# Thitrongdan202/Digital-Watermarking-for-image-Video-using-DCT-SVD-Singular-Value-Decomposition

Hardware: AMD Instinct MI355X
Metric: frames/sec embed+extract @4K Y-channel (higher is better)
Workload: dtype f32

## Files before the change

__graft_entry__.py:

```python
from __future__ import annotations

import importlib
import os
import subprocess
import sys

ROOT = os.path.dirname(os.path.abspath(__file__))
PKG_NAME = "digital-watermarking-for-image-video-using-dct-svd-singular-value-decomposition_amd"
CSRC = os.path.join(ROOT, PKG_NAME, "csrc")
LIB = os.path.join(CSRC, "libwmhip.so")
HARNESS_SRC = os.path.join(ROOT, "tests", "host_harness.cpp")
HARNESS_LIB = os.path.join(ROOT, "tests", "_build", "libwm_hostharness.so")

if ROOT not in sys.path:
    sys.path.insert(0, ROOT)


def _newer(target: str, *sources: str) -> bool:
    if not os.path.exists(target):
        return False
    t = os.path.getmtime(target)
    return all(os.path.getmtime(s) <= t for s in sources if os.path.exists(s))


def _run(cmd):
    r = subprocess.run(cmd, stdout=subprocess.PIPE, stderr=subprocess.STDOUT, text=True)
    if r.returncode != 0:
        raise RuntimeError("build failed: " + " ".join(cmd) + "\n" + r.stdout[-4000:])
    return r.stdout


def build_hip(force: bool = False) -> str:
    units = [os.path.join(CSRC, u) for u in ("wmhip.hip", "wm_ref.hip", "wm_pixel.hip", "wm_route.hip", "wm_enhance.hip")]
    deps = units + [os.path.join(CSRC, "wm_tile_math.h"), os.path.join(CSRC, "wm_enhance_math.h"), os.path.join(CSRC, "wm_internal.h"),
                    os.path.join(CSRC, "wm_jacobi_gfx950.inc"), os.path.join(CSRC, "wm_jacobi_v_gfx950.inc"),
                    os.path.join(CSRC, "wm_completion_tables.inc"), os.path.join(CSRC, "wm_ref_hier.inc"),
                    os.path.join(ROOT, "include", "wmhip.h")]
    if force or not _newer(LIB, *deps):
        hipcc = os.environ.get("HIPCC", "/opt/rocm/bin/hipcc")
        _run([hipcc, "-O3", "--offload-arch=gfx950", "-shared", "-fPIC", "-o", LIB] + units)
    return LIB


NOASM_LIB = os.path.join(ROOT, "tests", "_build", "libwmhip_noasm.so")


def build_hip_noasm(force: bool = False) -> str:
    os.makedirs(os.path.dirname(NOASM_LIB), exist_ok=True)
    units = [os.path.join(CSRC, u) for u in ("wmhip.hip", "wm_ref.hip", "wm_pixel.hip", "wm_route.hip", "wm_enhance.hip")]
    deps = units + [os.path.join(CSRC, "wm_tile_math.h"), os.path.join(CSRC, "wm_enhance_math.h"), os.path.join(CSRC, "wm_internal.h"),
                    os.path.join(CSRC, "wm_completion_tables.inc"), os.path.join(CSRC, "wm_ref_hier.inc"),
                    os.path.join(ROOT, "include", "wmhip.h")]
    if force or not _newer(NOASM_LIB, *deps):
        hipcc = os.environ.get("HIPCC", "/opt/rocm/bin/hipcc")
        _run([hipcc, "-O3", "--offload-arch=gfx950", "-shared", "-fPIC", "-DWM_NO_ASM_JACOBI", "-o", NOASM_LIB] + units)
    return NOASM_LIB


def build_host_harness(force: bool = False) -> str:
    os.makedirs(os.path.dirname(HARNESS_LIB), exist_ok=True)
    srcs = [HARNESS_SRC, os.path.join(CSRC, "wm_tile_math.h"), os.path.join(CSRC, "wm_completion_tables.inc")]
    if force or not _newer(HARNESS_LIB, *srcs):
        _run(["g++", "-O2", "-shared", "-fPIC", "-o", HARNESS_LIB, HARNESS_SRC])
    return HARNESS_LIB


MASK_HARNESS_SRC = os.path.join(ROOT, "tests", "mask_harness.cpp")


def build_mask_harness(sanitize: bool = False, force: bool = False) -> str:
    exe = os.path.join(ROOT, "tests", "_build", "mask_harness_san" if sanitize else "mask_harness")
    os.makedirs(os.path.dirname(exe), exist_ok=True)
    if force or not _newer(exe, MASK_HARNESS_SRC, os.path.join(CSRC, "wm_tile_math.h")):
        flags = ["-O1", "-g", "-fsanitize=address,undefined", "-fno-sanitize-recover=all"] if sanitize else ["-O2"]
        _run(["g++"] + flags + ["-o", exe, MASK_HARNESS_SRC])
    return exe


PAYLOAD_HARNESS_SRC = os.path.join(ROOT, "tests", "payload_harness.cpp")


def build_payload_harness(sanitize: bool = False, force: bool = False) -> str:
    exe = os.path.join(ROOT, "tests", "_build", "payload_harness_san" if sanitize else "payload_harness")
    os.makedirs(os.path.dirname(exe), exist_ok=True)
    if force or not _newer(exe, PAYLOAD_HARNESS_SRC, os.path.join(CSRC, "wm_tile_math.h")):
        flags = ["-O1", "-g", "-fsanitize=address,undefined", "-fno-sanitize-recover=all"] if sanitize else ["-O2"]
        _run(["g++"] + flags + ["-o", exe, PAYLOAD_HARNESS_SRC])
    return exe


PAYLOAD_DITHER_HARNESS_SRC = os.path.join(ROOT, "tests", "payload_dither_harness.cpp")


def build_payload_dither_harness(sanitize: bool = False, force: bool = False) -> str:
    exe = os.path.join(ROOT, "tests", "_build", "payload_dither_harness_san" if sanitize else "payload_dither_harness")
    os.makedirs(os.path.dirname(exe), exist_ok=True)
    if force or not _newer(exe, PAYLOAD_DITHER_HARNESS_SRC, os.path.join(CSRC, "wm_tile_math.h")):
        flags = ["-O1", "-g", "-fsanitize=address,undefined", "-fno-sanitize-recover=all"] if sanitize else ["-O2"]
        _run(["g++"] + flags + ["-o", exe, PAYLOAD_DITHER_HARNESS_SRC])
    return exe


PAYLOAD_SYNC_HARNESS_SRC = os.path.join(ROOT, "tests", "payload_sync_harness.cpp")


def build_payload_sync_harness(sanitize: bool = False, force: bool = False) -> str:
    exe = os.path.join(ROOT, "tests", "_build", "payload_sync_harness_san" if sanitize else "payload_sync_harness")
    os.makedirs(os.path.dirname(exe), exist_ok=True)
    if force or not _newer(exe, PAYLOAD_SYNC_HARNESS_SRC, os.path.join(CSRC, "wm_tile_math.h")):
        flags = ["-O1", "-g", "-fsanitize=address,undefined", "-fno-sanitize-recover=all"] if sanitize else ["-O2"]
        _run(["g++"] + flags + ["-o", exe, PAYLOAD_SYNC_HARNESS_SRC])
    return exe


def build() -> None:
    build_hip()
    build_hip_noasm()
    build_host_harness()
    build_mask_harness()
    build_mask_harness(sanitize=True)
# ... 49 lines not shown
```

digital-watermarking-for-image-video-using-dct-svd-singular-value-decomposition_amd/csrc/wm_jacobi_gfx950.inc:

```
__device__ __forceinline__ unsigned long long jacobi_cols_gfx950(const uint32_t (&lo)[8], const uint32_t (&hi)[8],
                                                                 wm::v2f (&a)[4][8], float (&n2)[8], const float conv2,
                                                                 const float skip2, const int min_sweeps,
                                                                 const int skip_from) {
  unsigned long long more;
  asm volatile(
      "s_mov_b32 s82, 0\n\t"
      "s_mov_b32 s83, 0x219392ef\n\t"
      "s_mov_b32 s84, %[conv]\n\t"
      "s_mov_b32 s85, %[skip]\n\t"
      "s_mov_b32 s86, %[minsw]\n\t"
      "s_mov_b32 s87, %[skipfrom]\n\t"
      "v_cvt_f32_ubyte0_e32 v40, %[lo0]\n\t"
      "v_cvt_f32_ubyte1_e32 v42, %[lo0]\n\t"
      "v_cvt_f32_ubyte2_e32 v44, %[lo0]\n\t"
      "v_cvt_f32_ubyte3_e32 v46, %[lo0]\n\t"
      "v_cvt_f32_ubyte0_e32 v48, %[hi0]\n\t"
      "v_cvt_f32_ubyte1_e32 v50, %[hi0]\n\t"
      "v_cvt_f32_ubyte2_e32 v52, %[hi0]\n\t"
      "v_cvt_f32_ubyte3_e32 v54, %[hi0]\n\t"
      "v_cvt_f32_ubyte0_e32 v41, %[lo1]\n\t"
      "v_cvt_f32_ubyte1_e32 v43, %[lo1]\n\t"
      "v_cvt_f32_ubyte2_e32 v45, %[lo1]\n\t"
      "v_cvt_f32_ubyte3_e32 v47, %[lo1]\n\t"
      "v_cvt_f32_ubyte0_e32 v49, %[hi1]\n\t"
      "v_cvt_f32_ubyte1_e32 v51, %[hi1]\n\t"
      "v_cvt_f32_ubyte2_e32 v53, %[hi1]\n\t"
      "v_cvt_f32_ubyte3_e32 v55, %[hi1]\n\t"
      "v_cvt_f32_ubyte0_e32 v56, %[lo2]\n\t"
      "v_cvt_f32_ubyte1_e32 v58, %[lo2]\n\t"
      "v_cvt_f32_ubyte2_e32 v60, %[lo2]\n\t"
      "v_cvt_f32_ubyte3_e32 v62, %[lo2]\n\t"
      "v_cvt_f32_ubyte0_e32 v64, %[hi2]\n\t"
      "v_cvt_f32_ubyte1_e32 v66, %[hi2]\n\t"
      "v_cvt_f32_ubyte2_e32 v68, %[hi2]\n\t"
      "v_cvt_f32_ubyte3_e32 v70, %[hi2]\n\t"
      "v_cvt_f32_ubyte0_e32 v57, %[lo3]\n\t"
      "v_cvt_f32_ubyte1_e32 v59, %[lo3]\n\t"
      "v_cvt_f32_ubyte2_e32 v61, %[lo3]\n\t"
      "v_cvt_f32_ubyte3_e32 v63, %[lo3]\n\t"
      "v_cvt_f32_ubyte0_e32 v65, %[hi3]\n\t"
      "v_cvt_f32_ubyte1_e32 v67, %[hi3]\n\t"
      "v_cvt_f32_ubyte2_e32 v69, %[hi3]\n\t"
      "v_cvt_f32_ubyte3_e32 v71, %[hi3]\n\t"
      "v_cvt_f32_ubyte0_e32 v72, %[lo4]\n\t"
      "v_cvt_f32_ubyte1_e32 v74, %[lo4]\n\t"
      "v_cvt_f32_ubyte2_e32 v76, %[lo4]\n\t"
      "v_cvt_f32_ubyte3_e32 v78, %[lo4]\n\t"
      "v_cvt_f32_ubyte0_e32 v80, %[hi4]\n\t"
      "v_cvt_f32_ubyte1_e32 v82, %[hi4]\n\t"
      "v_cvt_f32_ubyte2_e32 v84, %[hi4]\n\t"
      "v_cvt_f32_ubyte3_e32 v86, %[hi4]\n\t"
      "v_cvt_f32_ubyte0_e32 v73, %[lo5]\n\t"
      "v_cvt_f32_ubyte1_e32 v75, %[lo5]\n\t"
      "v_cvt_f32_ubyte2_e32 v77, %[lo5]\n\t"
      "v_cvt_f32_ubyte3_e32 v79, %[lo5]\n\t"
      "v_cvt_f32_ubyte0_e32 v81, %[hi5]\n\t"
      "v_cvt_f32_ubyte1_e32 v83, %[hi5]\n\t"
      "v_cvt_f32_ubyte2_e32 v85, %[hi5]\n\t"
      "v_cvt_f32_ubyte3_e32 v87, %[hi5]\n\t"
      "v_cvt_f32_ubyte0_e32 v88, %[lo6]\n\t"
      "v_cvt_f32_ubyte1_e32 v90, %[lo6]\n\t"
      "v_cvt_f32_ubyte2_e32 v92, %[lo6]\n\t"
      "v_cvt_f32_ubyte3_e32 v94, %[lo6]\n\t"
      "v_cvt_f32_ubyte0_e32 v96, %[hi6]\n\t"
      "v_cvt_f32_ubyte1_e32 v98, %[hi6]\n\t"
      "v_cvt_f32_ubyte2_e32 v100, %[hi6]\n\t"
      "v_cvt_f32_ubyte3_e32 v102, %[hi6]\n\t"
      "v_cvt_f32_ubyte0_e32 v89, %[lo7]\n\t"
      "v_cvt_f32_ubyte1_e32 v91, %[lo7]\n\t"
      "v_cvt_f32_ubyte2_e32 v93, %[lo7]\n\t"
      "v_cvt_f32_ubyte3_e32 v95, %[lo7]\n\t"
      "v_cvt_f32_ubyte0_e32 v97, %[hi7]\n\t"
      "v_cvt_f32_ubyte1_e32 v99, %[hi7]\n\t"
      "v_cvt_f32_ubyte2_e32 v101, %[hi7]\n\t"
      "v_cvt_f32_ubyte3_e32 v103, %[hi7]\n\t"
      "v_pk_mul_f32 v[120:121], v[40:41], v[40:41]\n\t"
      "v_pk_mul_f32 v[122:123], v[56:57], v[56:57]\n\t"
      "v_pk_mul_f32 v[124:125], v[72:73], v[72:73]\n\t"
      "v_pk_mul_f32 v[126:127], v[88:89], v[88:89]\n\t"
      "v_pk_fma_f32 v[120:121], v[42:43], v[42:43], v[120:121]\n\t"
      "v_pk_fma_f32 v[122:123], v[58:59], v[58:59], v[122:123]\n\t"
      "v_pk_fma_f32 v[124:125], v[74:75], v[74:75], v[124:125]\n\t"
      "v_pk_fma_f32 v[126:127], v[90:91], v[90:91], v[126:127]\n\t"
      "v_pk_fma_f32 v[120:121], v[44:45], v[44:45], v[120:121]\n\t"
      "v_pk_fma_f32 v[122:123], v[60:61], v[60:61], v[122:123]\n\t"
      "v_pk_fma_f32 v[124:125], v[76:77], v[76:77], v[124:125]\n\t"
      "v_pk_fma_f32 v[126:127], v[92:93], v[92:93], v[126:127]\n\t"
      "v_pk_fma_f32 v[120:121], v[46:47], v[46:47], v[120:121]\n\t"
      "v_pk_fma_f32 v[122:123], v[62:63], v[62:63], v[122:123]\n\t"
      "v_pk_fma_f32 v[124:125], v[78:79], v[78:79], v[124:125]\n\t"
      "v_pk_fma_f32 v[126:127], v[94:95], v[94:95], v[126:127]\n\t"
      "v_pk_fma_f32 v[120:121], v[48:49], v[48:49], v[120:121]\n\t"
      "v_pk_fma_f32 v[122:123], v[64:65], v[64:65], v[122:123]\n\t"
      "v_pk_fma_f32 v[124:125], v[80:81], v[80:81], v[124:125]\n\t"
      "v_pk_fma_f32 v[126:127], v[96:97], v[96:97], v[126:127]\n\t"
      "v_pk_fma_f32 v[120:121], v[50:51], v[50:51], v[120:121]\n\t"
      "v_pk_fma_f32 v[122:123], v[66:67], v[66:67], v[122:123]\n\t"
      "v_pk_fma_f32 v[124:125], v[82:83], v[82:83], v[124:125]\n\t"
      "v_pk_fma_f32 v[126:127], v[98:99], v[98:99], v[126:127]\n\t"
      "v_pk_fma_f32 v[120:121], v[52:53], v[52:53], v[120:121]\n\t"
      "v_pk_fma_f32 v[122:123], v[68:69], v[68:69], v[122:123]\n\t"
      "v_pk_fma_f32 v[124:125], v[84:85], v[84:85], v[124:125]\n\t"
      "v_pk_fma_f32 v[126:127], v[100:101], v[100:101], v[126:127]\n\t"
      "v_pk_fma_f32 v[120:121], v[54:55], v[54:55], v[120:121]\n\t"
      "v_pk_fma_f32 v[122:123], v[70:71], v[70:71], v[122:123]\n\t"
      "v_pk_fma_f32 v[124:125], v[86:87], v[86:87], v[124:125]\n\t"
      "v_pk_fma_f32 v[126:127], v[102:103], v[102:103], v[126:127]\n\t"
      "v_max3_f32 v112, v120, v121, v122\n\t"
      "v_max3_f32 v113, v123, v124, v125\n\t"
      "v_max3_f32 v112, v126, v127, v112\n\t"
      "s_mov_b64 s[94:95], 0\n\t"
      "v_max_f32_e32 v112, v112, v113\n\t"
      "v_mov_b32_e32 v113, 0xf149f2ca\n\t"
      "v_cmp_eq_f32_e64 s[92:93], v120, v112\n\t"
      "s_andn2_b64 s[96:97], s[92:93], s[94:95]\n\t"
      "s_or_b64 s[94:95], s[94:95], s[92:93]\n\t"
      "v_cndmask_b32_e64 v120, v120, v113, s[96:97]\n\t"
      "v_cmp_eq_f32_e64 s[92:93], v121, v112\n\t"
      "s_andn2_b64 s[96:97], s[92:93], s[94:95]\n\t"
      "s_or_b64 s[94:95], s[94:95], s[92:93]\n\t"
      "v_cndmask_b32_e64 v121, v121, v113, s[96:97]\n\t"
      "v_cndmask_b32_e64 v104, v40, v41, s[96:97]\n\t"
      "v_cndmask_b32_e64 v105, v42, v43, s[96:97]\n\t"
      "v_cndmask_b32_e64 v106, v44, v45, s[96:97]\n\t"
      "v_cndmask_b32_e64 v107, v46, v47, s[96:97]\n\t"
      "v_cndmask_b32_e64 v108, v48, v49, s[96:97]\n\t"
      "v_cndmask_b32_e64 v109, v50, v51, s[96:97]\n\t"
      "v_cndmask_b32_e64 v110, v52, v53, s[96:97]\n\t"
      "v_cndmask_b32_e64 v111, v54, v55, s[96:97]\n\t"
      "v_cmp_eq_f32_e64 s[92:93], v122, v112\n\t"
      "s_andn2_b64 s[96:97], s[92:93], s[94:95]\n\t"
      "s_or_b64 s[94:95], s[94:95], s[92:93]\n\t"
      "v_cndmask_b32_e64 v122, v122, v113, s[96:97]\n\t"
      "v_cndmask_b32_e64 v104, v104, v56, s[96:97]\n\t"
      "v_cndmask_b32_e64 v105, v105, v58, s[96:97]\n\t"
      "v_cndmask_b32_e64 v106, v106, v60, s[96:97]\n\t"
      "v_cndmask_b32_e64 v107, v107, v62, s[96:97]\n\t"
      "v_cndmask_b32_e64 v108, v108, v64, s[96:97]\n\t"
      "v_cndmask_b32_e64 v109, v109, v66, s[96:97]\n\t"
      "v_cndmask_b32_e64 v110, v110, v68, s[96:97]\n\t"
      "v_cndmask_b32_e64 v111, v111, v70, s[96:97]\n\t"
      "v_cmp_eq_f32_e64 s[92:93], v123, v112\n\t"
      "s_andn2_b64 s[96:97], s[92:93], s[94:95]\n\t"
      "s_or_b64 s[94:95], s[94:95], s[92:93]\n\t"
      "v_cndmask_b32_e64 v123, v123, v113, s[96:97]\n\t"
      "v_cndmask_b32_e64 v104, v104, v57, s[96:97]\n\t"
      "v_cndmask_b32_e64 v105, v105, v59, s[96:97]\n\t"
      "v_cndmask_b32_e64 v106, v106, v61, s[96:97]\n\t"
      "v_cndmask_b32_e64 v107, v107, v63, s[96:97]\n\t"
      "v_cndmask_b32_e64 v108, v108, v65, s[96:97]\n\t"
      "v_cndmask_b32_e64 v109, v109, v67, s[96:97]\n\t"
      "v_cndmask_b32_e64 v110, v110, v69, s[96:97]\n\t"
      "v_cndmask_b32_e64 v111, v111, v71, s[96:97]\n\t"
      "v_cmp_eq_f32_e64 s[92:93], v124, v112\n\t"
      "s_andn2_b64 s[96:97], s[92:93], s[94:95]\n\t"
      "s_or_b64 s[94:95], s[94:95], s[92:93]\n\t"
      "v_cndmask_b32_e64 v124, v124, v113, s[96:97]\n\t"
      "v_cndmask_b32_e64 v104, v104, v72, s[96:97]\n\t"
      "v_cndmask_b32_e64 v105, v105, v74, s[96:97]\n\t"
      "v_cndmask_b32_e64 v106, v106, v76, s[96:97]\n\t"
      "v_cndmask_b32_e64 v107, v107, v78, s[96:97]\n\t"
      "v_cndmask_b32_e64 v108, v108, v80, s[96:97]\n\t"
      "v_cndmask_b32_e64 v109, v109, v82, s[96:97]\n\t"
      "v_cndmask_b32_e64 v110, v110, v84, s[96:97]\n\t"
      "v_cndmask_b32_e64 v111, v111, v86, s[96:97]\n\t"
      "v_cmp_eq_f32_e64 s[92:93], v125, v112\n\t"
      "s_andn2_b64 s[96:97], s[92:93], s[94:95]\n\t"
      "s_or_b64 s[94:95], s[94:95], s[92:93]\n\t"
      "v_cndmask_b32_e64 v125, v125, v113, s[96:97]\n\t"
      "v_cndmask_b32_e64 v104, v104, v73, s[96:97]\n\t"
      "v_cndmask_b32_e64 v105, v105, v75, s[96:97]\n\t"
      "v_cndmask_b32_e64 v106, v106, v77, s[96:97]\n\t"
      "v_cndmask_b32_e64 v107, v107, v79, s[96:97]\n\t"
      "v_cndmask_b32_e64 v108, v108, v81, s[96:97]\n\t"
      "v_cndmask_b32_e64 v109, v109, v83, s[96:97]\n\t"
      "v_cndmask_b32_e64 v110, v110, v85, s[96:97]\n\t"
      "v_cndmask_b32_e64 v111, v111, v87, s[96:97]\n\t"
      "v_cmp_eq_f32_e64 s[92:93], v126, v112\n\t"
      "s_andn2_b64 s[96:97], s[92:93], s[94:95]\n\t"
      "s_or_b64 s[94:95], s[94:95], s[92:93]\n\t"
      "v_cndmask_b32_e64 v126, v126, v113, s[96:97]\n\t"
      "v_cndmask_b32_e64 v104, v104, v88, s[96:97]\n\t"
      "v_cndmask_b32_e64 v105, v105, v90, s[96:97]\n\t"
      "v_cndmask_b32_e64 v106, v106, v92, s[96:97]\n\t"
      "v_cndmask_b32_e64 v107, v107, v94, s[96:97]\n\t"
      "v_cndmask_b32_e64 v108, v108, v96, s[96:97]\n\t"
      "v_cndmask_b32_e64 v109, v109, v98, s[96:97]\n\t"
      "v_cndmask_b32_e64 v110, v110, v100, s[96:97]\n\t"
      "v_cndmask_b32_e64 v111, v111, v102, s[96:97]\n\t"
      "v_cmp_eq_f32_e64 s[92:93], v127, v112\n\t"
// ... 4791 lines not shown
```

digital-watermarking-for-image-video-using-dct-svd-singular-value-decomposition_amd/csrc/wm_tile_math.h:

```cpp
#pragma once
#include <stdint.h>
#include <math.h>

#if defined(__HIPCC__)
#define WM_HD __host__ __device__ __forceinline__
#else
#define WM_HD inline
#endif

namespace wm {

WM_HD float frcp(float x) {
#if defined(__HIP_DEVICE_COMPILE__)
  return __builtin_amdgcn_rcpf(x);
#else
  return 1.0f / x;
#endif
}
WM_HD float frsq(float x) {
#if defined(__HIP_DEVICE_COMPILE__)
  return __builtin_amdgcn_rsqf(x);
#else
  return 1.0f / sqrtf(x);
#endif
}
WM_HD float fsqrt(float x) {
#if defined(__HIP_DEVICE_COMPILE__)
  return __builtin_amdgcn_sqrtf(x);
#else
  return sqrtf(x);
#endif
}
WM_HD float ffma(float a, float b, float c) {
#if defined(__HIP_DEVICE_COMPILE__)
  return __builtin_fmaf(a, b, c);
#else
  return fmaf(a, b, c);
#endif
}
WM_HD bool wave_any(bool p) {
#if defined(__HIP_DEVICE_COMPILE__)
  return __builtin_amdgcn_ballot_w64(p) != 0ull;
#else
  return p;
#endif
}

constexpr float C1 = 0.49039264020161522f;
constexpr float C2 = 0.46193976625564337f;
constexpr float C3 = 0.41573480615127262f;
constexpr float C4 = 0.35355339059327379f;
constexpr float C5 = 0.27778511650980114f;
constexpr float C6 = 0.19134171618254492f;
constexpr float C7 = 0.09754516100806417f;

WM_HD void dct8(float& x0, float& x1, float& x2, float& x3,
                float& x4, float& x5, float& x6, float& x7) {
  const float s0 = x0 + x7, s1 = x1 + x6, s2 = x2 + x5, s3 = x3 + x4;
  const float d0 = x0 - x7, d1 = x1 - x6, d2 = x2 - x5, d3 = x3 - x4;
  const float e0 = s0 + s3, e1 = s1 + s2, e2 = s0 - s3, e3 = s1 - s2;
  x0 = C4 * (e0 + e1);
  x4 = C4 * (e0 - e1);
  x2 = ffma(C2, e2, C6 * e3);
  x6 = ffma(C6, e2, -C2 * e3);
  x1 = ffma(C1, d0, ffma(C3, d1, ffma(C5, d2, C7 * d3)));
  x3 = ffma(C3, d0, ffma(-C7, d1, ffma(-C1, d2, -C5 * d3)));
  x5 = ffma(C5, d0, ffma(-C1, d1, ffma(C7, d2, C3 * d3)));
  x7 = ffma(C7, d0, ffma(-C5, d1, ffma(C3, d2, -C1 * d3)));
}

WM_HD void idct8(float& x0, float& x1, float& x2, float& x3,
                 float& x4, float& x5, float& x6, float& x7) {
  const float p = C4 * (x0 + x4), q = C4 * (x0 - x4);
  const float r = ffma(C2, x2, C6 * x6), t = ffma(C6, x2, -C2 * x6);
  const float e0 = p + r, e3 = p - r, e1 = q + t, e2 = q - t;
  const float o0 = ffma(C1, x1, ffma(C3, x3, ffma(C5, x5, C7 * x7)));
  const float o1 = ffma(C3, x1, ffma(-C7, x3, ffma(-C1, x5, -C5 * x7)));
  const float o2 = ffma(C5, x1, ffma(-C1, x3, ffma(C7, x5, C3 * x7)));
  const float o3 = ffma(C7, x1, ffma(-C5, x3, ffma(C3, x5, -C1 * x7)));
  x0 = e0 + o0; x7 = e0 - o0;
  x1 = e1 + o1; x6 = e1 - o1;
  x2 = e2 + o2; x5 = e2 - o2;
  x3 = e3 + o3; x4 = e3 - o3;
}

WM_HD void dct8x8(float (&a)[8][8]) {
#pragma unroll
  for (int c = 0; c < 8; ++c)
    dct8(a[0][c], a[1][c], a[2][c], a[3][c], a[4][c], a[5][c], a[6][c], a[7][c]);
#pragma unroll
  for (int r = 0; r < 8; ++r)
    dct8(a[r][0], a[r][1], a[r][2], a[r][3], a[r][4], a[r][5], a[r][6], a[r][7]);
}
WM_HD void idct8x8(float (&a)[8][8]) {
#pragma unroll
  for (int r = 0; r < 8; ++r)
    idct8(a[r][0], a[r][1], a[r][2], a[r][3], a[r][4], a[r][5], a[r][6], a[r][7]);
#pragma unroll
  for (int c = 0; c < 8; ++c)
    idct8(a[0][c], a[1][c], a[2][c], a[3][c], a[4][c], a[5][c], a[6][c], a[7][c]);
}

constexpr float JAC_TOL2 = 1e-15f;
constexpr float JAC_CONV2 = 1e-7f;
constexpr int JAC_MAX_SWEEPS = 12;
constexpr int JAC_DEFI_FROM = 6;
constexpr float JAC_CONV2_SIGMA = 1e-2f;
constexpr float JAC_MOVE2 = 1e-6f;
constexpr float JAC_SKIP2 = 1e-12f;

template <bool WITH_V>
WM_HD void jacobi_rot(float (&a)[8][8], float (&v)[8][8], float (&n2)[8],
                      const int p, const int q, bool& notconv) {
  float g = a[0][p] * a[0][q];
#pragma unroll
  for (int r = 1; r < 8; ++r) g = ffma(a[r][p], a[r][q], g);
  const float al = n2[p], be = n2[q];
  const float ab = al * be, gg = g * g;
  const bool big = gg > JAC_TOL2 * ab;
  notconv = notconv || (gg > JAC_CONV2 * ab);
  const float tau = be - al, g2 = g + g;
  const float h = fsqrt(ffma(tau, tau, g2 * g2));
  float t = g2 * frcp(fabsf(tau) + h);
  t = (tau < 0.0f) ? -t : t;
  t = big ? t : 0.0f;
  const float c = frsq(ffma(t, t, 1.0f)), s = c * t;
  const float tg = t * g;
  const float aln = al - tg, ben = be + tg;
  const bool sw = tau > 0.0f;
  const float C = sw ? s : c, S = sw ? -c : s;
  n2[p] = sw ? ben : aln;
  n2[q] = sw ? aln : ben;
#pragma unroll
  for (int r = 0; r < 8; ++r) {
    const float x = a[r][p], y = a[r][q];
    a[r][p] = ffma(C, x, -S * y);
    a[r][q] = ffma(S, x, C * y);
  }
  if (WITH_V) {
#pragma unroll
    for (int r = 0; r < 8; ++r) {
      const float x = v[r][p], y = v[r][q];
      v[r][p] = ffma(C, x, -S * y);
      v[r][q] = ffma(S, x, C * y);
    }
  }
}

WM_HD void col_norms2(const float (&a)[8][8], float (&n2)[8]) {
#pragma unroll
  for (int c = 0; c < 8; ++c) {
    float s = a[0][c] * a[0][c];
#pragma unroll
    for (int r = 1; r < 8; ++r) s = ffma(a[r][c], a[r][c], s);
    n2[c] = s;
  }
}

template <bool WITH_V>
WM_HD int jacobi_svd8(float (&a)[8][8], float (&v)[8][8], float (&n2)[8], float (&vn2)[8]) {
  if (WITH_V) {
#pragma unroll
    for (int r = 0; r < 8; ++r)
#pragma unroll
      for (int c = 0; c < 8; ++c) v[r][c] = (r == c) ? 1.0f : 0.0f;
  }
  int sweep = 0;
  bool more = true;
  while (more && sweep < JAC_MAX_SWEEPS) {
    col_norms2(a, n2);
    bool notconv = false;
#pragma unroll
    for (int p = 0; p < 7; ++p)
#pragma unroll
      for (int q = p + 1; q < 8; ++q) jacobi_rot<WITH_V>(a, v, n2, p, q, notconv);
    ++sweep;
    more = wave_any(notconv);
  }
  col_norms2(a, n2);
  if (WITH_V) col_norms2(v, vn2);
  else {
#pragma unroll
    for (int c = 0; c < 8; ++c) vn2[c] = 1.0f;
  }
  return more ? -sweep : sweep;
}

typedef float v2f __attribute__((vector_size(8)));

// ... 34 lines not shown
  x3 = e3 + o3; x4 = e3 - o3;
}
WM_HD void dct8x8_to_pk(const float (&a)[8][8], v2f (&b)[4][8]) {
#pragma unroll
  for (int c = 0; c < 8; ++c) {
    float x0 = a[0][c], x1 = a[1][c], x2 = a[2][c], x3 = a[3][c], x4 = a[4][c], x5 = a[5][c], x6 = a[6][c], x7 = a[7][c];
    dct8(x0, x1, x2, x3, x4, x5, x6, x7);
    const v2f p0 = {x0, x1}, p1 = {x2, x3}, p2 = {x4, x5}, p3 = {x6, x7};
    b[0][c] = p0; b[1][c] = p1; b[2][c] = p2; b[3][c] = p3;
  }
#pragma unroll
  for (int rp = 0; rp < 4; ++rp)
    dct8_pk(b[rp][0], b[rp][1], b[rp][2], b[rp][3], b[rp][4], b[rp][5], b[rp][6], b[rp][7]);
}
WM_HD void idct8x8_from_pk(v2f (&b)[4][8], float (&a)[8][8]) {
#pragma unroll
  for (int rp = 0; rp < 4; ++rp)
    idct8_pk(b[rp][0], b[rp][1], b[rp][2], b[rp][3], b[rp][4], b[rp][5], b[rp][6], b[rp][7]);
#pragma unroll
  for (int c = 0; c < 8; ++c) {
    float x0 = b[0][c][0], x1 = b[0][c][1], x2 = b[1][c][0], x3 = b[1][c][1];
    float x4 = b[2][c][0], x5 = b[2][c][1], x6 = b[3][c][0], x7 = b[3][c][1];
    idct8(x0, x1, x2, x3, x4, x5, x6, x7);
    a[0][c] = x0; a[1][c] = x1; a[2][c] = x2; a[3][c] = x3; a[4][c] = x4; a[5][c] = x5; a[6][c] = x6; a[7][c] = x7;
  }
}

template <int HALF>
WM_HD v2f fma2_bcast(const v2f ab, const v2f x, v2f acc) {
#if defined(__HIP_DEVICE_COMPILE__)
  if (HALF == 0) asm("v_pk_fma_f32 %0, %1, %2, %0 op_sel_hi:[0,1,1]" : "+v"(acc) : "v"(ab), "v"(x));
  else asm("v_pk_fma_f32 %0, %1, %2, %0 op_sel:[1,0,0]" : "+v"(acc) : "v"(ab), "v"(x));
  return acc;
#else
  return fma2(splat2(ab[HALF]), x, acc);
#endif
}
template <int HALF>
WM_HD v2f mul2_bcast(const v2f ab, const v2f x) {
#if defined(__HIP_DEVICE_COMPILE__)
  v2f r;
  if (HALF == 0) asm("v_pk_mul_f32 %0, %1, %2 op_sel_hi:[0,1]" : "=v"(r) : "v"(ab), "v"(x));
  else asm("v_pk_mul_f32 %0, %1, %2 op_sel:[1,0]" : "=v"(r) : "v"(ab), "v"(x));
  return r;
#else
  return splat2(ab[HALF]) * x;
#endif
}

constexpr float SIGMA_RATIO_MIN2 = 1e-10f;

template <int CHECK, bool SKIP = false>
WM_HD void jacobi_rot_pk(v2f (&a)[4][8], float (&n2)[8], const int p, const int q, bool& notconv) {
  v2f gv = a[0][p] * a[0][q];
#pragma unroll
  for (int rp = 1; rp < 4; ++rp) gv = fma2(a[rp][p], a[rp][q], gv);
  const float g = gv[0] + gv[1];
  const float al = n2[p], be = n2[q];
  if (CHECK) notconv = notconv || (g * g > (CHECK == 2 ? JAC_CONV2_SIGMA : JAC_CONV2) * (al * be));
  if (SKIP && !wave_any(g * g > JAC_SKIP2 * (al * be))) return;
  const float tau = be - al;
  const float ta = fabsf(tau) + 1e-18f;
  const float g2 = g + g;
  const float ih = frsq(ffma(g2, g2, ta * ta));
  const float x = ffma(0.5f * ta, ih, 0.5f);
  const float rx = frsq(x);
  const float c0 = x * rx;
  const float s0 = (g * ih) * rx;
  const bool sw = tau > 0.0f;
  const float C = sw ? s0 : c0, Sn = sw ? c0 : s0;
  const float w = fabsf((s0 * rx) * g);
  if (CHECK) notconv = notconv || (w * w > (JAC_MOVE2 * fmaxf(al, be)) * n2[0]);
  n2[p] = fmaxf(al, be) + w;
  n2[q] = fminf(al, be) - w;
  const v2f Cv = splat2(C), Sv = splat2(Sn);
#pragma unroll
  for (int rp = 0; rp < 4; ++rp) {
    const v2f X = a[rp][p], Y = a[rp][q];
    a[rp][p] = fma2(Cv, X, Sv * Y);
    a[rp][q] = fma2(Cv, Y, -(Sv * X));
  }
}

WM_HD void jacobi_rot_scaled_pk(v2f (&a)[4][8], float (&n2)[8], float (&w2)[8], const int p, const int q, const bool wave_swaps) {
  v2f gv = a[0][p] * a[0][q];
#pragma unroll
  for (int rp = 1; rp < 4; ++rp) gv = fma2(a[rp][p], a[rp][q], gv);
  const float gt = gv[0] + gv[1];
  const float al = n2[p], be = n2[q];
  const float gg = (gt * (w2[p] * w2[q])) * gt;
  const float tau = be - al;
  const float ta = fabsf(tau) + 1e-18f;
  const float ih = frsq(ffma(gg, 4.0f, ta * ta));
  const float x = ffma(0.5f * ta, ih, 0.5f);
  const float rx = frsq(x);
  const float u = gt * ih;
  const float gh = gg * ih;
  if (!wave_swaps) {
    const float rx2 = rx * rx;
    const float tq = u * w2[p];
    const float v = u * rx2;
    const float w = gh * rx2;
    w2[p] *= x;
    const float tp = v * w2[q];
    w2[q] *= rx2;
    const v2f Tp = splat2(tp), Tq = splat2(-tq);
#pragma unroll
    for (int rp = 0; rp < 4; ++rp) {
      a[rp][p] = fma2(Tp, a[rp][q], a[rp][p]);
      a[rp][q] = fma2(Tq, a[rp][p], a[rp][q]);
    }
    n2[p] = al + w;
    n2[q] = be - w;
  } else {
    const float pq = w2[p] * w2[q];
    const float c0 = x * rx;
    const float r = frsq(pq);
    const float w = (gh * rx) * rx;
    const float s0 = (u * rx) * (pq * r);
    const float rq = w2[q] * r, rp_ = w2[p] * r;
    const bool sw = tau > 0.0f;
    const float Sn = sw ? c0 : s0, C = sw ? s0 : c0;
    const v2f Cv = splat2(C), Sp = splat2(Sn * rq), Sq = splat2(Sn * rp_);
#pragma unroll
    for (int rp = 0; rp < 4; ++rp) {
      const v2f X = a[rp][p], Y = a[rp][q];
      a[rp][p] = fma2(Cv, X, Sp * Y);
      a[rp][q] = fma2(Cv, Y, -(Sq * X));
    }
    n2[p] = fmaxf(al, be) + w;
    n2[q] = fminf(al, be) - w;
  }
}

WM_HD void col_norms2_pk(const v2f (&a)[4][8], float (&n2)[8]) {
#pragma unroll
  for (int c = 0; c < 8; ++c) {
    v2f s = a[0][c] * a[0][c];
#pragma unroll
    for (int rp = 1; rp < 4; ++rp) s = fma2(a[rp][c], a[rp][c], s);
    n2[c] = s[0] + s[1];
  }
}

template <int CHECK, bool SKIP = false>
WM_HD void jacobi_sweep_pk(v2f (&a)[4][8], float (&n2)[8], bool& notconv) {
#pragma unroll
  for (int p = 0; p < 7; ++p)
#pragma unroll
    for (int q = p + 1; q < 8; ++q) jacobi_rot_pk<CHECK, SKIP>(a, n2, p, q, notconv);
}
WM_HD void jacobi_sweep_scaled_pk(v2f (&a)[4][8], float (&n2)[8], float (&w2)[8]) {
#pragma unroll
  for (int p = 0; p < 7; ++p)
#pragma unroll
    for (int q = p + 1; q < 8; ++q) jacobi_rot_scaled_pk(a, n2, w2, p, q, wave_any(n2[q] - n2[p] > 0.0f));
}
WM_HD void col_norms2_scaled_pk(const v2f (&a)[4][8], const float (&w2)[8], float (&n2)[8]) {
  col_norms2_pk(a, n2);
#pragma unroll
  for (int c = 0; c < 8; ++c) n2[c] *= w2[c];
}
WM_HD void fold_scales_pk(v2f (&a)[4][8], const float (&w2)[8]) {
#pragma unroll
  for (int c = 0; c < 8; ++c) {
    const v2f d = splat2(w2[c] * frsq(w2[c]));
#pragma unroll
    for (int rp = 0; rp < 4; ++rp) a[rp][c] = d * a[rp][c];
  }
}

WM_HD float fmax3(const float a, const float b, const float c) { return fmaxf(fmaxf(a, b), c); }
WM_HD void lq_prelude_pk(v2f (&a)[4][8]) {
  v2f rn[4];
#pragma unroll
  for (int c = 0; c < 8; ++c)
#pragma unroll
    for (int rp = 0; rp < 4; ++rp) rn[rp] = (c == 0) ? a[rp][c] * a[rp][c] : fma2(a[rp][c], a[rp][c], rn[rp]);
#pragma unroll
  for (int k = 0; k < 7; ++k) {
    float m = fmax3(rn[0][0], rn[0][1], rn[1][0]);
    const float m2 = fmax3(rn[1][1], rn[2][0], rn[2][1]);
    m = fmaxf(fmax3(rn[3][0], rn[3][1], m), m2);
    float x[8];
    bool found = false;
#pragma unroll
    for (int r = 0; r < 8; ++r) {
      const bool hit = rn[r >> 1][r & 1] == m;
      const bool mine = hit && !found;
      found = found || hit;
      rn[r >> 1][r & 1] = mine ? -1e30f : rn[r >> 1][r & 1];
      if (r) {
#pragma unroll
        for (int c = k; c < 8; ++c) x[c] = mine ? a[r >> 1][c][r & 1] : (r == 1 ? a[0][c][0] : x[c]);
      }
    }
    float t2 = x[7] * x[7];
#pragma unroll
    for (int c = 6; c > k; --c) t2 = ffma(x[c], x[c], t2);
    const float nx2 = ffma(x[k], x[k], t2);
    const float nrm = copysignf(nx2 * frsq(fmaxf(1e-36f, nx2)), x[k]);
    const float vk = x[k] + nrm;
    const float sb = frsq(fmaxf(1e-36f, 0.5f * ffma(vk, vk, t2)));
    x[k] = vk;
#pragma unroll
    for (int c = k; c < 8; ++c) x[c] *= sb;
    v2f w[4];
#pragma unroll
    for (int c = k; c < 8; ++c)
#pragma unroll
      for (int rp = 0; rp < 4; ++rp) w[rp] = (c == k) ? splat2(x[c]) * a[rp][c] : fma2(splat2(x[c]), a[rp][c], w[rp]);
#pragma unroll
    for (int c = k; c < 8; ++c)
#pragma unroll
      for (int rp = 0; rp < 4; ++rp) a[rp][c] = fma2(splat2(x[c]), -w[rp], a[rp][c]);
    if (k < 6) {
#pragma unroll
      for (int rp = 0; rp < 4; ++rp) rn[rp] = fma2(-a[rp][k], a[rp][k], rn[rp]);
    }
  }
}

template <bool SIGMA_ONLY = false>
WM_HD int jacobi_cols_pk(v2f (&a)[4][8], float (&n2)[8]) {
  lq_prelude_pk(a);
  bool notconv = false;
  float w2[8] = {1.0f, 1.0f, 1.0f, 1.0f, 1.0f, 1.0f, 1.0f, 1.0f};
  col_norms2_pk(a, n2);
  jacobi_sweep_scaled_pk(a, n2, w2);
  jacobi_sweep_scaled_pk(a, n2, w2);
  int sweep = 2;
  if (!SIGMA_ONLY) {
    col_norms2_scaled_pk(a, w2, n2);
    jacobi_sweep_scaled_pk(a, n2, w2);
    sweep = 3;
  }
  fold_scales_pk(a, w2);
  bool more = true;
  while (more && sweep < JAC_MAX_SWEEPS) {
    if ((sweep & 1) == 0) col_norms2_pk(a, n2);
    notconv = false;
    if (!SIGMA_ONLY) jacobi_sweep_pk<1, true>(a, n2, notconv);
    else jacobi_sweep_pk<2>(a, n2, notconv);
    ++sweep;
    if (sweep >= JAC_DEFI_FROM && !(n2[7] > SIGMA_RATIO_MIN2 * n2[0])) notconv = false;
    more = wave_any(notconv);
  }
  col_norms2_pk(a, n2);
  return more ? -sweep : sweep;
}

struct RawTile { uint32_t lo[8], hi[8]; };

WM_HD float raw_px(const RawTile& t, const int r, const int c) {
  const uint32_t w = (c < 4) ? t.lo[r] : t.hi[r];
  return (float)((w >> (8 * (c & 3))) & 0xffu);
}
WM_HD void raw_to_pk(const RawTile& t, v2f (&a)[4][8]) {
#pragma unroll
  for (int rp = 0; rp < 4; ++rp)
#pragma unroll
    for (int c = 0; c < 8; ++c) {
      v2f v = {raw_px(t, 2 * rp, c), raw_px(t, 2 * rp + 1, c)};
      a[rp][c] = v;
    }
}
WM_HD void raw_to_f32(const RawTile& t, float (&a)[8][8]) {
#pragma unroll
  for (int r = 0; r < 8; ++r)
#pragma unroll
    for (int c = 0; c < 8; ++c) a[r][c] = raw_px(t, r, c);
}

WM_HD int sigma_tile_pk(const RawTile& t, float (&s)[8]) {
  v2f a[4][8];
  float n2[8];
  raw_to_pk(t, a);
  const int sweeps = jacobi_cols_pk<true>(a, n2);
#pragma unroll
  for (int i = 0; i < 8; ++i) s[i] = fsqrt(n2[i]);
  return sweeps;
}

WM_HD uint32_t quant_u8(float x) {
  x = fminf(fmaxf(x, 0.0f), 255.0f);
  return (uint32_t)x;
}

WM_HD int embed_jacobi_pk(const RawTile& t, v2f (&a)[4][8], float (&n2)[8]) {
  raw_to_pk(t, a);
  return jacobi_cols_pk(a, n2);
}

WM_HD void embed_coeffs_pk(const float (&n2)[8], const float (&sw)[8], const float (&alpha_k)[8],
                           float (&e)[8], float (&sc)[8], bool& deficient) {
  deficient = !(n2[7] > SIGMA_RATIO_MIN2 * n2[0]);
#pragma unroll
  for (int i = 0; i < 8; ++i) {
    const float rs = frsq(fmaxf(n2[i], 1e-30f));
    sc[i] = n2[i] * rs;
    e[i] = (alpha_k[i] * sw[i]) * (rs * rs * rs);
  }
}

template <bool YW>
WM_HD void embed_half_pk(const uint32_t (&w)[8], const v2f (&a)[4][8], const float (&e)[8],
                         uint32_t (&outw)[8], float* yw, const size_t yw_stride) {
#pragma unroll
  for (int r = 0; r < 8; ++r) outw[r] = 0u;
#pragma unroll
  for (int cp = 0; cp < 2; ++cp) {
    const int sh = 16 * cp;
    v2f g[8];
#pragma unroll
    for (int r = 0; r < 8; ++r) {
      const uint32_t ww = w[r] >> sh;
      const v2f x = {(float)(ww & 0xffu), (float)((ww >> 8) & 0xffu)};
#pragma unroll
      for (int i = 0; i < 8; ++i) {
        const v2f ab = a[r >> 1][i];
        if (r == 0) g[i] = mul2_bcast<0>(ab, x);
        else g[i] = (r & 1) ? fma2_bcast<1>(ab, x, g[i]) : fma2_bcast<0>(ab, x, g[i]);
      }
    }
#pragma unroll
    for (int i = 0; i < 8; ++i) g[i] = g[i] * splat2(e[i]);
#pragma unroll
    for (int r = 0; r < 8; ++r) {
      const uint32_t ww = w[r] >> sh;
      v2f y = {(float)(ww & 0xffu), (float)((ww >> 8) & 0xffu)};
#pragma unroll
// ... 683 lines not shown
```

digital-watermarking-for-image-video-using-dct-svd-singular-value-decomposition_amd/csrc/wmhip.hip:

```cpp
#include <hip/hip_runtime.h>
#include <stdio.h>
#include <stdlib.h>
#include <string.h>
#include <new>

#include "wm_internal.h"
#include "wm_tile_math.h"

using namespace wmi;

namespace wmi {

thread_local char g_err[512] = "";

int set_err(int code, const char* fmt, const char* a, const char* b) {
  snprintf(g_err, sizeof(g_err), fmt, a, b);
  return code;
}

int grow(wm_ctx* ctx, void** buf, size_t* have, size_t bytes, const char* what) {
  if (bytes <= *have) return WM_OK;
  if (*buf) {
    WM_HIP(hipStreamSynchronize(ctx->stream));
    WM_HIP(hipFree(*buf));
    *buf = nullptr; *have = 0;
  }
  const size_t mb = (size_t)1 << 20;
  const size_t want = (bytes + mb - 1) / mb * mb;
  if (hipMalloc(buf, want) != hipSuccess) {
    (void)hipGetLastError();
    *buf = nullptr;
    return set_err(WM_ERR_NOMEM, "hipMalloc failed for %s", what);
  }
  *have = want;
  return WM_OK;
}

}

namespace {

constexpr int N_SUMS = 5;

#if !defined(WM_NO_ASM_JACOBI)
#include "wm_jacobi_gfx950.inc"
#endif

__device__ __forceinline__ int sigma_tile_dev(const wm::RawTile& raw, float (&s)[8]) {
#if !defined(WM_NO_ASM_JACOBI)
  wm::v2f a[4][8];
  float n2[8];
  constexpr float SIGMA_SKIP2 = 1e-8f;
  constexpr int SIGMA_SKIP_FROM = 2;
  const unsigned long long more = jacobi_cols_gfx950(raw.lo, raw.hi, a, n2, wm::JAC_CONV2_SIGMA, SIGMA_SKIP2, 3, SIGMA_SKIP_FROM);
#pragma unroll
  for (int i = 0; i < 8; ++i) s[i] = wm::fsqrt(n2[i]);
  return more ? -1 : 1;
#else
  return wm::sigma_tile_pk(raw, s);
#endif
}

template <bool ALIGNED>
__device__ __forceinline__ uint32_t load_px4(const uint8_t* __restrict__ q) {
  if (ALIGNED) return *reinterpret_cast<const uint32_t*>(q);
  return q[0] | (q[1] << 8) | (q[2] << 16) | ((uint32_t)q[3] << 24);
}
template <bool ALIGNED>
__device__ __forceinline__ void store_px4(uint8_t* __restrict__ q, const uint32_t w) {
  if (ALIGNED) { *reinterpret_cast<uint32_t*>(q) = w; return; }
#pragma unroll
  for (int i = 0; i < 4; ++i) q[i] = (uint8_t)(w >> (8 * i));
}
template <bool ALIGNED>
__device__ __forceinline__ void load_px8(const uint8_t* __restrict__ q, uint32_t& lo, uint32_t& hi) {
  if (ALIGNED) { const uint2 w = *reinterpret_cast<const uint2*>(q); lo = w.x; hi = w.y; }
  else { lo = load_px4<false>(q); hi = load_px4<false>(q + 4); }
}
template <bool ALIGNED>
__device__ __forceinline__ void store_px8(uint8_t* __restrict__ q, const uint32_t lo, const uint32_t hi) {
  if (ALIGNED) *reinterpret_cast<uint2*>(q) = make_uint2(lo, hi);
  else { store_px4<false>(q, lo); store_px4<false>(q + 4, hi); }
}

template <bool ALIGNED>
__device__ __forceinline__ void load_raw(const uint8_t* __restrict__ p, const size_t stride, wm::RawTile& t) {
#pragma unroll
  for (int r = 0; r < 8; ++r) load_px8<ALIGNED>(p + r * stride, t.lo[r], t.hi[r]);
}

template <bool ALIGNED>
__device__ __forceinline__ void load_tile_u8(const uint8_t* __restrict__ p, const size_t stride, float (&a)[8][8]) {
#pragma unroll
  for (int r = 0; r < 8; ++r) {
    uint32_t lo, hi;
    load_px8<ALIGNED>(p + r * stride, lo, hi);
    a[r][0] = (float)(lo & 0xffu); a[r][1] = (float)((lo >> 8) & 0xffu);
    a[r][2] = (float)((lo >> 16) & 0xffu); a[r][3] = (float)(lo >> 24);
    a[r][4] = (float)(hi & 0xffu); a[r][5] = (float)((hi >> 8) & 0xffu);
    a[r][6] = (float)((hi >> 16) & 0xffu); a[r][7] = (float)(hi >> 24);
  }
}

template <bool ALIGNED>
__device__ __forceinline__ void store_tile_u8(uint8_t* __restrict__ p, const size_t stride, const float (&a)[8][8]) {
#pragma unroll
  for (int r = 0; r < 8; ++r) {
    const uint32_t lo = wm::quant_u8(a[r][0]) | (wm::quant_u8(a[r][1]) << 8) |
                        (wm::quant_u8(a[r][2]) << 16) | (wm::quant_u8(a[r][3]) << 24);
    const uint32_t hi = wm::quant_u8(a[r][4]) | (wm::quant_u8(a[r][5]) << 8) |
                        (wm::quant_u8(a[r][6]) << 16) | (wm::quant_u8(a[r][7]) << 24);
    store_px8<ALIGNED>(p + r * stride, lo, hi);
  }
}

template <bool ALIGNED>
__device__ __forceinline__ void load_words(const uint8_t* __restrict__ p, const size_t stride, uint32_t (&w)[8]) {
#pragma unroll
  for (int r = 0; r < 8; ++r) w[r] = load_px4<ALIGNED>(p + r * stride);
}
template <bool ALIGNED>
__device__ __forceinline__ void store_words(uint8_t* __restrict__ p, const size_t stride, const uint32_t (&w)[8]) {
#pragma unroll
  for (int r = 0; r < 8; ++r) store_px4<ALIGNED>(p + r * stride, w[r]);
}

template <bool VEC>
__device__ __forceinline__ void load_row8_f32(const float* __restrict__ p, float (&row)[8]) {
  if (VEC) {
    const float4 x = *reinterpret_cast<const float4*>(p);
    const float4 y = *reinterpret_cast<const float4*>(p + 4);
    row[0] = x.x; row[1] = x.y; row[2] = x.z; row[3] = x.w;
    row[4] = y.x; row[5] = y.y; row[6] = y.z; row[7] = y.w;
  } else {
#pragma unroll
    for (int i = 0; i < 8; ++i) row[i] = p[i];
  }
// ... 1844 lines not shown
```

Before: 23420.

## Add sigma-only Jacobi asm kernel and compute initial column norms with integer dot4

Moves the sigma-only tile path to a new generated assembly kernel that returns only the column norms, without producing the rotated matrix. The initial squared column norms are computed directly from packed uint8 pixels with v_dot4_u32_u8 and then converted to float, replacing a chain of packed float FMAs. The portable sigma path now keeps the column scales unfolded through the later sweeps, folds them at a fixed sweep, and uses a reciprocal and an inline convergence test. This aims to cut ALU work and register pressure in the sigma SVD. The risks are a generated include that may not exist at build time and small numeric differences from the changed convergence behaviour.

```diff
diff --git a/__graft_entry__.py b/__graft_entry__.py
--- a/__graft_entry__.py
+++ b/__graft_entry__.py
@@ -33,9 +33,15 @@
 def build_hip(force: bool = False) -> str:
     units = [os.path.join(CSRC, u) for u in ("wmhip.hip", "wm_ref.hip", "wm_pixel.hip", "wm_route.hip", "wm_enhance.hip")]
     deps = units + [os.path.join(CSRC, "wm_tile_math.h"), os.path.join(CSRC, "wm_enhance_math.h"), os.path.join(CSRC, "wm_internal.h"),
-                    os.path.join(CSRC, "wm_jacobi_gfx950.inc"), os.path.join(CSRC, "wm_jacobi_v_gfx950.inc"),
+                    os.path.join(CSRC, "wm_jacobi_gfx950.inc"), os.path.join(CSRC, "wm_jacobi_sigma_gfx950.inc"),
+                    os.path.join(CSRC, "wm_jacobi_v_gfx950.inc"),
                     os.path.join(CSRC, "wm_completion_tables.inc"), os.path.join(CSRC, "wm_ref_hier.inc"),
                     os.path.join(ROOT, "include", "wmhip.h")]
+    sys.path.insert(0, os.path.join(ROOT, "tools"))
+    try:
+        importlib.import_module("gen_jacobi_asm").write_sigma()
+    finally:
+        sys.path.remove(os.path.join(ROOT, "tools"))
     if force or not _newer(LIB, *deps):
         hipcc = os.environ.get("HIPCC", "/opt/rocm/bin/hipcc")
         _run([hipcc, "-O3", "--offload-arch=gfx950", "-shared", "-fPIC", "-o", LIB] + units)
diff --git a/digital-watermarking-for-image-video-using-dct-svd-singular-value-decomposition_amd/csrc/wm_jacobi_gfx950.inc b/digital-watermarking-for-image-video-using-dct-svd-singular-value-decomposition_amd/csrc/wm_jacobi_gfx950.inc
--- a/digital-watermarking-for-image-video-using-dct-svd-singular-value-decomposition_amd/csrc/wm_jacobi_gfx950.inc
+++ b/digital-watermarking-for-image-video-using-dct-svd-singular-value-decomposition_amd/csrc/wm_jacobi_gfx950.inc
@@ -74,38 +74,30 @@
       "v_cvt_f32_ubyte1_e32 v99, %[hi7]\n\t"
       "v_cvt_f32_ubyte2_e32 v101, %[hi7]\n\t"
       "v_cvt_f32_ubyte3_e32 v103, %[hi7]\n\t"
-      "v_pk_mul_f32 v[120:121], v[40:41], v[40:41]\n\t"
-      "v_pk_mul_f32 v[122:123], v[56:57], v[56:57]\n\t"
-      "v_pk_mul_f32 v[124:125], v[72:73], v[72:73]\n\t"
-      "v_pk_mul_f32 v[126:127], v[88:89], v[88:89]\n\t"
-      "v_pk_fma_f32 v[120:121], v[42:43], v[42:43], v[120:121]\n\t"
-      "v_pk_fma_f32 v[122:123], v[58:59], v[58:59], v[122:123]\n\t"
-      "v_pk_fma_f32 v[124:125], v[74:75], v[74:75], v[124:125]\n\t"
-      "v_pk_fma_f32 v[126:127], v[90:91], v[90:91], v[126:127]\n\t"
-      "v_pk_fma_f32 v[120:121], v[44:45], v[44:45], v[120:121]\n\t"
-      "v_pk_fma_f32 v[122:123], v[60:61], v[60:61], v[122:123]\n\t"
-      "v_pk_fma_f32 v[124:125], v[76:77], v[76:77], v[124:125]\n\t"
-      "v_pk_fma_f32 v[126:127], v[92:93], v[92:93], v[126:127]\n\t"
-      "v_pk_fma_f32 v[120:121], v[46:47], v[46:47], v[120:121]\n\t"
-      "v_pk_fma_f32 v[122:123], v[62:63], v[62:63], v[122:123]\n\t"
-      "v_pk_fma_f32 v[124:125], v[78:79], v[78:79], v[124:125]\n\t"
-      "v_pk_fma_f32 v[126:127], v[94:95], v[94:95], v[126:127]\n\t"
-      "v_pk_fma_f32 v[120:121], v[48:49], v[48:49], v[120:121]\n\t"
-      "v_pk_fma_f32 v[122:123], v[64:65], v[64:65], v[122:123]\n\t"
-      "v_pk_fma_f32 v[124:125], v[80:81], v[80:81], v[124:125]\n\t"
-      "v_pk_fma_f32 v[126:127], v[96:97], v[96:97], v[126:127]\n\t"
-      "v_pk_fma_f32 v[120:121], v[50:51], v[50:51], v[120:121]\n\t"
-      "v_pk_fma_f32 v[122:123], v[66:67], v[66:67], v[122:123]\n\t"
-      "v_pk_fma_f32 v[124:125], v[82:83], v[82:83], v[124:125]\n\t"
-      "v_pk_fma_f32 v[126:127], v[98:99], v[98:99], v[126:127]\n\t"
-      "v_pk_fma_f32 v[120:121], v[52:53], v[52:53], v[120:121]\n\t"
-      "v_pk_fma_f32 v[122:123], v[68:69], v[68:69], v[122:123]\n\t"
-      "v_pk_fma_f32 v[124:125], v[84:85], v[84:85], v[124:125]\n\t"
-      "v_pk_fma_f32 v[126:127], v[100:101], v[100:101], v[126:127]\n\t"
-      "v_pk_fma_f32 v[120:121], v[54:55], v[54:55], v[120:121]\n\t"
-      "v_pk_fma_f32 v[122:123], v[70:71], v[70:71], v[122:123]\n\t"
-      "v_pk_fma_f32 v[124:125], v[86:87], v[86:87], v[124:125]\n\t"
-      "v_pk_fma_f32 v[126:127], v[102:103], v[102:103], v[126:127]\n\t"
+      "v_dot4_u32_u8 v120, %[lo0], %[lo0], 0\n\t"
+      "v_dot4_u32_u8 v121, %[lo1], %[lo1], 0\n\t"
+      "v_dot4_u32_u8 v122, %[lo2], %[lo2], 0\n\t"
+      "v_dot4_u32_u8 v123, %[lo3], %[lo3], 0\n\t"
+      "v_dot4_u32_u8 v124, %[lo4], %[lo4], 0\n\t"
+      "v_dot4_u32_u8 v125, %[lo5], %[lo5], 0\n\t"
+      "v_dot4_u32_u8 v126, %[lo6], %[lo6], 0\n\t"
+      "v_dot4_u32_u8 v127, %[lo7], %[lo7], 0\n\t"
+      "v_dot4_u32_u8 v120, %[hi0], %[hi0], v120\n\t"
+      "v_dot4_u32_u8 v121, %[hi1], %[hi1], v121\n\t"
+      "v_dot4_u32_u8 v122, %[hi2], %[hi2], v122\n\t"
+      "v_dot4_u32_u8 v123, %[hi3], %[hi3], v123\n\t"
+      "v_dot4_u32_u8 v124, %[hi4], %[hi4], v124\n\t"
+      "v_dot4_u32_u8 v125, %[hi5], %[hi5], v125\n\t"
+      "v_dot4_u32_u8 v126, %[hi6], %[hi6], v126\n\t"
+      "v_dot4_u32_u8 v127, %[hi7], %[hi7], v127\n\t"
+      "v_cvt_f32_u32_e32 v120, v120\n\t"
+      "v_cvt_f32_u32_e32 v121, v121\n\t"
+      "v_cvt_f32_u32_e32 v122, v122\n\t"
+      "v_cvt_f32_u32_e32 v123, v123\n\t"
+      "v_cvt_f32_u32_e32 v124, v124\n\t"
+      "v_cvt_f32_u32_e32 v125, v125\n\t"
+      "v_cvt_f32_u32_e32 v126, v126\n\t"
+      "v_cvt_f32_u32_e32 v127, v127\n\t"
       "v_max3_f32 v112, v120, v121, v122\n\t"
       "v_max3_f32 v113, v123, v124, v125\n\t"
       "v_max3_f32 v112, v126, v127, v112\n\t"
diff --git a/digital-watermarking-for-image-video-using-dct-svd-singular-value-decomposition_amd/csrc/wm_tile_math.h b/digital-watermarking-for-image-video-using-dct-svd-singular-value-decomposition_amd/csrc/wm_tile_math.h
--- a/digital-watermarking-for-image-video-using-dct-svd-singular-value-decomposition_amd/csrc/wm_tile_math.h
+++ b/digital-watermarking-for-image-video-using-dct-svd-singular-value-decomposition_amd/csrc/wm_tile_math.h
@@ -105,6 +105,7 @@
 constexpr float JAC_CONV2 = 1e-7f;
 constexpr int JAC_MAX_SWEEPS = 12;
 constexpr int JAC_DEFI_FROM = 6;
+constexpr int JAC_SIGMA_FOLD_AT = 6;
 constexpr float JAC_CONV2_SIGMA = 1e-2f;
 constexpr float JAC_MOVE2 = 1e-6f;
 constexpr float JAC_SKIP2 = 1e-12f;
@@ -305,22 +306,24 @@
   }
 }
 
-WM_HD void jacobi_rot_scaled_pk(v2f (&a)[4][8], float (&n2)[8], float (&w2)[8], const int p, const int q, const bool wave_swaps) {
+template <bool TESTED, bool RCP>
+WM_HD void jacobi_rot_scaled_pk(v2f (&a)[4][8], float (&n2)[8], float (&w2)[8], const int p, const int q, const bool wave_swaps,
+                                bool& notconv) {
   v2f gv = a[0][p] * a[0][q];
 #pragma unroll
   for (int rp = 1; rp < 4; ++rp) gv = fma2(a[rp][p], a[rp][q], gv);
   const float gt = gv[0] + gv[1];
   const float al = n2[p], be = n2[q];
   const float gg = (gt * (w2[p] * w2[q])) * gt;
+  if (TESTED) notconv = notconv || (gg > JAC_CONV2_SIGMA * (al * be));
   const float tau = be - al;
   const float ta = fabsf(tau) + 1e-18f;
   const float ih = frsq(ffma(gg, 4.0f, ta * ta));
   const float x = ffma(0.5f * ta, ih, 0.5f);
-  const float rx = frsq(x);
   const float u = gt * ih;
   const float gh = gg * ih;
   if (!wave_swaps) {
-    const float rx2 = rx * rx;
+    const float rx2 = RCP ? frcp(x) : frsq(x) * frsq(x);
     const float tq = u * w2[p];
     const float v = u * rx2;
     const float w = gh * rx2;
@@ -333,9 +336,11 @@
       a[rp][p] = fma2(Tp, a[rp][q], a[rp][p]);
       a[rp][q] = fma2(Tq, a[rp][p], a[rp][q]);
     }
+    if (TESTED) notconv = notconv || (w * w > (JAC_MOVE2 * al) * n2[0]);
     n2[p] = al + w;
     n2[q] = be - w;
   } else {
+    const float rx = frsq(x);
     const float pq = w2[p] * w2[q];
     const float c0 = x * rx;
     const float r = frsq(pq);
@@ -351,10 +356,15 @@
       a[rp][p] = fma2(Cv, X, Sp * Y);
       a[rp][q] = fma2(Cv, Y, -(Sq * X));
     }
+    if (TESTED) notconv = notconv || (w * w > (JAC_MOVE2 * fmaxf(al, be)) * n2[0]);
     n2[p] = fmaxf(al, be) + w;
     n2[q] = fminf(al, be) - w;
   }
 }
+WM_HD void jacobi_rot_scaled_pk(v2f (&a)[4][8], float (&n2)[8], float (&w2)[8], const int p, const int q, const bool wave_swaps) {
+  bool unused = false;
+  jacobi_rot_scaled_pk<false, false>(a, n2, w2, p, q, wave_swaps, unused);
+}
 
 WM_HD void col_norms2_pk(const v2f (&a)[4][8], float (&n2)[8]) {
 #pragma unroll
@@ -373,11 +383,19 @@
 #pragma unroll
     for (int q = p + 1; q < 8; ++q) jacobi_rot_pk<CHECK, SKIP>(a, n2, p, q, notconv);
 }
+template <bool RCP = false>
 WM_HD void jacobi_sweep_scaled_pk(v2f (&a)[4][8], float (&n2)[8], float (&w2)[8]) {
+  bool unused = false;
 #pragma unroll
   for (int p = 0; p < 7; ++p)
 #pragma unroll
-    for (int q = p + 1; q < 8; ++q) jacobi_rot_scaled_pk(a, n2, w2, p, q, wave_any(n2[q] - n2[p] > 0.0f));
+    for (int q = p + 1; q < 8; ++q) jacobi_rot_scaled_pk<false, RCP>(a, n2, w2, p, q, wave_any(n2[q] - n2[p] > 0.0f), unused);
+}
+WM_HD void jacobi_sweep_scaled_tested_pk(v2f (&a)[4][8], float (&n2)[8], float (&w2)[8], bool& notconv) {
+#pragma unroll
+  for (int p = 0; p < 7; ++p)
+#pragma unroll
+    for (int q = p + 1; q < 8; ++q) jacobi_rot_scaled_pk<true, true>(a, n2, w2, p, q, wave_any(n2[q] - n2[p] > 0.0f), notconv);
 }
 WM_HD void col_norms2_scaled_pk(const v2f (&a)[4][8], const float (&w2)[8], float (&n2)[8]) {
   col_norms2_pk(a, n2);
@@ -450,26 +468,39 @@
   bool notconv = false;
   float w2[8] = {1.0f, 1.0f, 1.0f, 1.0f, 1.0f, 1.0f, 1.0f, 1.0f};
   col_norms2_pk(a, n2);
-  jacobi_sweep_scaled_pk(a, n2, w2);
-  jacobi_sweep_scaled_pk(a, n2, w2);
+  jacobi_sweep_scaled_pk<SIGMA_ONLY>(a, n2, w2);
+  jacobi_sweep_scaled_pk<SIGMA_ONLY>(a, n2, w2);
   int sweep = 2;
   if (!SIGMA_ONLY) {
     col_norms2_scaled_pk(a, w2, n2);
     jacobi_sweep_scaled_pk(a, n2, w2);
     sweep = 3;
   }
-  fold_scales_pk(a, w2);
+  if (!SIGMA_ONLY) fold_scales_pk(a, w2);
   bool more = true;
   while (more && sweep < JAC_MAX_SWEEPS) {
-    if ((sweep & 1) == 0) col_norms2_pk(a, n2);
+    if ((sweep & 1) == 0) {
+      if (SIGMA_ONLY && sweep == JAC_SIGMA_FOLD_AT) {
+        fold_scales_pk(a, w2);
+#pragma unroll
+        for (int c = 0; c < 8; ++c) w2[c] = 1.0f;
+      }
+      if (SIGMA_ONLY) col_norms2_scaled_pk(a, w2, n2);
+      else col_norms2_pk(a, n2);
+    }
     notconv = false;
     if (!SIGMA_ONLY) jacobi_sweep_pk<1, true>(a, n2, notconv);
-    else jacobi_sweep_pk<2>(a, n2, notconv);
+    else jacobi_sweep_scaled_tested_pk(a, n2, w2, notconv);
     ++sweep;
     if (sweep >= JAC_DEFI_FROM && !(n2[7] > SIGMA_RATIO_MIN2 * n2[0])) notconv = false;
     more = wave_any(notconv);
   }
-  col_norms2_pk(a, n2);
+  if (SIGMA_ONLY) {
+    col_norms2_scaled_pk(a, w2, n2);
+    fold_scales_pk(a, w2);
+  } else {
+    col_norms2_pk(a, n2);
+  }
   return more ? -sweep : sweep;
 }
 
diff --git a/digital-watermarking-for-image-video-using-dct-svd-singular-value-decomposition_amd/csrc/wmhip.hip b/digital-watermarking-for-image-video-using-dct-svd-singular-value-decomposition_amd/csrc/wmhip.hip
--- a/digital-watermarking-for-image-video-using-dct-svd-singular-value-decomposition_amd/csrc/wmhip.hip
+++ b/digital-watermarking-for-image-video-using-dct-svd-singular-value-decomposition_amd/csrc/wmhip.hip
@@ -44,15 +44,18 @@
 
 #if !defined(WM_NO_ASM_JACOBI)
 #include "wm_jacobi_gfx950.inc"
+#if !__has_include("wm_jacobi_sigma_gfx950.inc")
+#error "wm_jacobi_sigma_gfx950.inc is generated: run `python tools/gen_jacobi_asm.py --write` (build() does) before compiling"
+#endif
+#include "wm_jacobi_sigma_gfx950.inc"
 #endif
 
 __device__ __forceinline__ int sigma_tile_dev(const wm::RawTile& raw, float (&s)[8]) {
 #if !defined(WM_NO_ASM_JACOBI)
-  wm::v2f a[4][8];
   float n2[8];
   constexpr float SIGMA_SKIP2 = 1e-8f;
   constexpr int SIGMA_SKIP_FROM = 2;
-  const unsigned long long more = jacobi_cols_gfx950(raw.lo, raw.hi, a, n2, wm::JAC_CONV2_SIGMA, SIGMA_SKIP2, 3, SIGMA_SKIP_FROM);
+  const unsigned long long more = jacobi_sigma_gfx950(raw.lo, raw.hi, n2, wm::JAC_CONV2_SIGMA, SIGMA_SKIP2, 3, SIGMA_SKIP_FROM);
 #pragma unroll
   for (int i = 0; i < 8; ++i) s[i] = wm::fsqrt(n2[i]);
   return more ? -1 : 1;
```

New measurement: 23720 (median of 6 runs). +1.3%, better.
